# LenShustek/readtape

Hardware: AMD Instinct MI355X
Metric: Msamples/sec (all tracks) 9-trk TBIN (higher is better)
Workload: dtype i16/f32; 1 GPU; C2: synthetic 9-track 800 BPI NRZI, 781.25 kHz, 1 parmset; rows_per_gpu=101799450, rows_total=101799450, bytes_per_gpu=1832390100, parmsets=1

## Files before the change

### readtape_amd/csrc/rtfe_api.hip

```cpp
#include <hip/hip_runtime.h>

#include <limits.h>
#include <math.h>
#include <stdarg.h>
#include <stdio.h>
#include <stdlib.h>
#include <string.h>

#include <mutex>

#include "rt_frontend.h"
#include "rtfe_device.h"

#include "rtfe_sift.hip"
#include "rtfe_kernels.hip"
#include "rtfe_zeros.hip"
#include "rtfe_diffz.hip"
#include "rtfe_ww.hip"
#include "rtfe_gain.hip"
#include "rtfe_dense.hip"
#include "rtfe_pack.hip"
#include "rtfe_csv.hip"
#include "rtfe_csvout.hip"
#include "rtfe_textfile.hip"
// ... 565 lines not shown
   void t1(int k) { t1s(k, st); }
   void skip_rest() {
      unsigned mask = 0;
      for (int k = 0; k < kNumKernels; ++k) if (ran[k]) mask |= 1u << k;
      if (h->timing) h->ev_ran[evset] = mask;
      for (int k = 0; k < kNumKernels; ++k) if (!ran[k]) { t0(k); t1(k); } }
   void launch_bursts(hipStream_t s) {
      const int wpr_env = h->bursts_wpr;
      const int wpr = (wpr_env >= 1 && wpr_env <= kBrWords) ? wpr_env : kBrWords;
      const long long rounds = (L.nwords + wpr - 1) / wpr;
      if ((wpr_env > 0 || rounds >= 3) && rounds <= kBrRoundsMax && d.debug != 5) {
         hipLaunchKernelGGL(k_bursts_cnt, dim3((unsigned)rounds), dim3(1024), 0, s, (const unsigned long long *)w.qwords, L.nwords, nchunks, wpr, d.gap_chunks, a.first_is_tape_start, maxb, w.rtot);
         hipLaunchKernelGGL(k_bursts_emit, dim3((unsigned)rounds), dim3(1024), 0, s, (const unsigned long long *)w.qwords, L.nwords, nchunks, nrows, wpr, d.gap_chunks, a.first_is_tape_start, a.d_bursts, maxb, (const uint32_t *)w.rtot);
         hipLaunchKernelGGL(k_bursts_tail, dim3(1), dim3(1024), 0, s, (int)rounds, (const uint32_t *)w.rtot, nrows, (long long)a.own_rows, d.ntrks, d.gap_chunks,
                            d.cap_frac, d.nparm, (long long)a.event_capacity, a.d_bursts, maxb, w.scratch, a.d_nbursts); }
      else
         hipLaunchKernelGGL(k_bursts, dim3(1), dim3(1024), 0, s, (const unsigned long long *)w.qwords, L.nwords, nchunks, nrows, (long long)a.own_rows, d.ntrks,
                            d.gap_chunks, a.first_is_tape_start, d.cap_frac, d.nparm, (long long)a.event_capacity, a.d_bursts, maxb, w.scratch, a.d_nbursts, d.debug == 5 ? 1 : 0); }
   void launch_zones(hipStream_t s) {
      hipLaunchKernelGGL(k_zones, dim3(h->num_cus * 8), dim3(64), 0, s, h->d_dev, a.d_rows, nrows, (const rtfe_burst *)a.d_bursts, (const BurstScratch *)w.scratch, w.ctl);
      if (d.invert)
         hipLaunchKernelGGL(k_rails, dim3(h->num_cus * 8), dim3(64), 0, s, h->d_dev, a.d_rows, nrows, (const rtfe_burst *)a.d_bursts, (const BurstScratch *)w.scratch, w.ctl); }
   void launch_decode(int mode) {
      const DecodePlan dp = decode_plan(h);
      t0(kTDecode);
      hipLaunchKernelGGL(k_decode, dim3(h->num_cus * dp.per_cu), dim3(dp.threads), h->lds_bytes, st, h->d_dev, a.d_rows, nrows,
                         row_base, a.d_bursts, w.scratch, a.d_counts, a.d_events, 0xffffffffu, 0, 0, mode, w.ctl);
      t1(kTDecode); }
   void launch_sift() {
      t0(kTSift);
      const sfs_kernel_t sfs = sf_special(h);
      const int pthreads = sfs ? sfs_threads(d) : sf_threads(d), plds = sfs ? sfs_lds(d) : d.pk_lds;
      int spc = lds_wgs_per_cu(plds, 512, 32 / (pthreads / 64));
      if (h->sift_wgs >= 1 && h->sift_wgs < spc) spc = h->sift_wgs;
      if (spc < 1) spc = 1;
      long long pgrid = (long long)h->num_cus * spc;
      if (pgrid > L.ptiles) pgrid = L.ptiles;
      if (sfs) {
         for (int sc = 0; sc < d.nscreens; ++sc) {
            SfArgs sa;
            sa.rows = a.d_rows; sa.nrows = nrows; sa.ntiles = (int)L.ptiles; sa.qtile = sc == 0 ? w.qtile : nullptr; sa.dir = w.dir; sa.pool = w.pool; sa.hard = w.hard; sa.hard_cap = L.hard_cap;
            sa.hard_count = &w.scratch->hard_count; sa.dbg = w.scratch->scr; sa.hcap = d.pk_slot; sa.wave_cap = d.pk_wave_cap; sa.invert = d.invert;
            sa.quiet_i = d.quiet_i; sa.cfg = h->d_dev; sa.hi_i = d.screen[sc].sure_i;
            sa.cut = d.cut; sa.debug = d.debug; sa.defer = 1; sa.nscreens = d.nscreens; sa.sc = sc;
            const int lds_sc = sfs_lds_sc(d, sc);
            int spc_sc = lds_wgs_per_cu(lds_sc, 512, spc);
            if (h->sfs_occ[sc] >= 1 && spc_sc > h->sfs_occ[sc]) spc_sc = h->sfs_occ[sc];
            if (spc_sc < 1) spc_sc = 1;
            long long grid_sc = (long long)h->num_cus * spc_sc;
            if (grid_sc > L.ptiles) grid_sc = L.ptiles;
            hipLaunchKernelGGL(sf_special_sc(h, sc), dim3((unsigned)grid_sc), dim3(pthreads), lds_sc, st, sa); } }
      else {
         const sf_kernel_t sfk = sf_kernel(sf_wmax(d), pthreads, sf_nv(d));
         hipLaunchKernelGGL(sfk, dim3((unsigned)pgrid), dim3(pthreads), d.pk_lds, st, (const DevCfg *)h->d_dev, a.d_rows, nrows, L.ptiles,
                            w.qtile, w.dir, w.pool, w.hard, L.hard_cap, &w.scratch->hard_count, w.scratch->scr); }
      t1(kTSift); }
   void launch_streams() {
      t0(kTPrep);
      const int nlists = d.nscreens * d.ntrks;
      const int nsc = (int)((L.ptiles + 1023) / 1024);
      hipLaunchKernelGGL(k_sift_hard, dim3(h->num_cus * 16), dim3(256), 0, st, (const DevCfg *)h->d_dev, a.d_rows, nrows, (const SfHard *)w.hard, L.hard_cap,
                         (const int *)&w.scratch->hard_count, w.ovf, w.extra, w.scratch->dbg2);
      hipLaunchKernelGGL(k_pscan1, dim3(nsc), dim3(1024), 0, st, (const PeakDir *)w.dir, (const int *)w.extra, (int)L.ptiles, nlists, w.tstart, w.ctotc);
      hipLaunchKernelGGL(k_pscan2, dim3(1), dim3(1024), 0, st, nsc, nlists, (const uint32_t *)w.ctotc, w.coff, w.ctot);
      PrepArgs ppa; ppa.nlists = nlists; ppa.ntrks = d.ntrks; ppa.hcap = d.pk_slot; ppa.run = h->prep_run; ppa.mv = d.maxvolts;
      hipLaunchKernelGGL(k_prep, dim3(h->num_cus * (h->prep_wgs >= 1 && h->prep_wgs <= 4096 ? h->prep_wgs : 32)), dim3(256), 0, st, ppa, (const PeakDir *)w.dir, (const unsigned char *)w.pool, (const unsigned char *)w.ovf,
                         (const uint32_t *)w.tstart, (const uint32_t *)w.coff, (const uint32_t *)w.ctot, L.ptiles, L.ccap, w.crec, w.eref, w.work, L.work_cap, &w.scratch->prep_work);
      hipLaunchKernelGGL(k_clear, dim3(h->num_cus * 4), dim3(256), 0, st, (const unsigned long long *)w.work, L.work_cap, (const int *)&w.scratch->prep_work, (const uint32_t *)w.ctot, L.ccap, w.crec);
#ifdef RTFE_CPU_EMUL
      if (getenv("RTFE_PREP_CHECK")) hipLaunchKernelGGL(k_prep_check, dim3(1), dim3(64), 0, st, (const DevCfg *)h->d_dev, (const uint32_t *)w.ctot, L.ccap, (const CRec *)w.crec);
      if (getenv("RTFE_PREP_CHECK") && atoi(getenv("RTFE_PREP_CHECK")) > 1)
         hipLaunchKernelGGL(k_prep_shapes, dim3(1), dim3(64), 0, st, nlists, (int)d.pk_slot, h->prep_run, L.ptiles, L.ccap, (const PeakDir *)w.dir, (const unsigned char *)w.pool, (const uint32_t *)w.ctot);
#endif
      t1(kTPrep); }
   void launch_chains() {
      t0(kTGain);
      for (int mode = 0; mode < 2; ++mode) {
         if (mode == 1) t0(kTGainTail);
         hipLaunchKernelGGL(k_gain, dim3(h->num_cus * 4), dim3(64), 0, st, (const DevCfg *)h->d_dev, mode, w.cst, nrows, row_base, (const rtfe_burst *)a.d_bursts,
                            w.scratch, w.ctl, a.d_counts, a.d_events, w.chain, (const CRec *)w.crec, (const uint2 *)w.eref, (const uint32_t *)w.tstart, (const uint32_t *)w.coff, (const uint32_t *)w.ctot, L.ccap,
                            (const unsigned char *)w.pool, L.ptiles, w.segs, L.seg_cap, a.d_rows);
         if (mode == 0) {
            t1(kTGain); t0(kTGainS);
            hipLaunchKernelGGL(k_gain_seg, dim3(h->num_cus * 16), dim3(64), 0, st, (const DevCfg *)h->d_dev, (const ChainSt *)w.cst, w.scratch, (const CRec *)w.crec, L.ccap, w.segs, (const int *)&w.scratch->nsegs, L.seg_cap, w.gfire);
            hipLaunchKernelGGL(k_gain_join, dim3(h->num_cus * 2), dim3(64), 0, st, (const DevCfg *)h->d_dev, w.cst, (const rtfe_burst *)a.d_bursts, w.scratch, (const BurstCtl *)w.ctl, a.d_counts, w.chain, w.segs);
            t1(kTGainS); } }
#ifdef RTFE_CPU_EMUL
      if (getenv("RTFE_PREP_CHECK") && atoi(getenv("RTFE_PREP_CHECK")) > 1 && d.pk_seg_recs > 0)
         hipLaunchKernelGGL(k_seg_shapes, dim3(1), dim3(64), 0, st, (const DevCfg *)h->d_dev, (const ChainSt *)w.cst, (const BurstScratch *)w.scratch, (const CRec *)w.crec, L.ccap,
                            (const GsSeg *)w.segs, L.seg_cap, (const float *)w.gfire);
#endif
      t1(kTGainTail); }
   void launch_emit(hipStream_t side) {
      t0(kTEmit);
      hipStream_t se = st;
      if (side != st) { se = side; (void)hipEventRecord(h->ev_fork2, st); (void)hipStreamWaitEvent(se, h->ev_fork2, 0); }
      hipLaunchKernelGGL(k_emit, dim3(h->num_cus * 32), dim3(64), 0, se, h->d_dev, (const rtfe_burst *)a.d_bursts, (const BurstScratch *)w.scratch, (const BurstCtl *)w.ctl, (const uint32_t *)a.d_counts, a.d_events,
                         (const float *)w.chain, (const CRec *)w.crec, (const uint2 *)w.eref, L.ccap, (const unsigned char *)w.pool, (const ChainSt *)w.cst, a.d_rows, nrows, (const GsSeg *)w.segs);
      if (se != st) (void)hipEventRecord(h->ev_join2, se);
      hipLaunchKernelGGL(k_emit_seg, dim3(h->num_cus * 16), dim3(256), 0, st, (const DevCfg *)h->d_dev, (const ChainSt *)w.cst, (const BurstCtl *)w.ctl, a.d_events, (const CRec *)w.crec, (const uint2 *)w.eref, L.ccap,
                         (const unsigned char *)w.pool, (const GsSeg *)w.segs, (const int *)&w.scratch->nsegs, L.seg_cap, (const float *)w.gfire, (int)(L.max_bursts * d.nparm * d.ntrks), a.d_rows, nrows);
      if (se != st) (void)hipStreamWaitEvent(st, h->ev_join2, 0);
      hipLaunchKernelGGL(k_publish, dim3(h->num_cus < 64 ? h->num_cus : 64), dim3(256), 0, st, h->d_dev, nrows, a.d_bursts, w.scratch, w.ctl);
      if (d.nuset < d.nparm)
         hipLaunchKernelGGL(k_dup_sets, dim3(h->num_cus * 8), dim3(256), 0, st, (const DevCfg *)h->d_dev, (const rtfe_burst *)a.d_bursts, (const BurstScratch *)w.scratch, (const BurstCtl *)w.ctl, a.d_counts, a.d_events);
      t1(kTEmit); }
   void launch_peak_path() {
      const int stop_after = h->peak_stop;
      uint4 *const extra16 = ws_at<uint4>(a.d_workspace, L.extra);
      hipLaunchKernelGGL(k_scan_begin, dim3(h->num_cus * 4), dim3(256), 0, st, h->d_dev, w.scratch, extra16, (long long)((L.cst - L.extra) / 16), a.d_rows, nrows);
      launch_sift();
      hipStream_t sa = st;
      if (h->overlap && stop_after >= 99) {
         ensure_side(h);
         if (h->side) { sa = h->side; (void)hipEventRecord(h->ev_fork, st); (void)hipStreamWaitEvent(sa, h->ev_fork, 0); } }
      t0s(kTBursts, sa);
      hipLaunchKernelGGL(k_qpack, dim3(h->num_cus < 64 ? h->num_cus : 64), dim3(256), 0, sa, (const uint16_t *)w.qtile, L.ptiles, w.qwords, L.nwords);
      launch_bursts(sa);
      if (stop_after >= 3) launch_zones(sa);
      t1s(kTBursts, sa);
      if (sa != st) (void)hipEventRecord(h->ev_join, sa);
      launch_streams();
      if (sa != st) (void)hipStreamWaitEvent(st, h->ev_join, 0);
      if (stop_after < 3) return;
      launch_chains();
      if (stop_after < 4) return;
      launch_emit(sa);
      if (stop_after < 5) return;
      launch_decode(kDecodeRedo);
      if (d.adapt_floor) hipLaunchKernelGGL(k_adapt_floor, dim3(1), dim3(1), 0, st, h->d_dev, (const BurstScratch *)w.scratch); }
   void launch_dense_path() {
      (void)hipMemsetAsync(w.scratch, 0, kScratchBytes, st);
      (void)hipMemsetAsync(w.qwords, 0, (size_t)L.nwords * 8, st);
      const int dlds = (int)ds_lds_layout(d.ntrks, d.halo_rows, d.ds_pad + kDsTile + kDsRight, d.ds_up).total + 64;
      int dpc = lds_wgs_per_cu(dlds, 1024, 8);
      if (h->dseg_wgs >= 1 && h->dseg_wgs < dpc) dpc = h->dseg_wgs;
      if (dpc < 1) dpc = 1;
      long long dg = (long long)h->num_cus * dpc;
      if (dg > L.dtiles) dg = L.dtiles;
      t0(kTDseg);
      int dthreads = kDsThreads;
      if (h->dseg_threads >= 64 && h->dseg_threads <= kDsThreads) dthreads = h->dseg_threads / 64 * 64;
      unsigned char *const qbytes = ws_at<unsigned char>(a.d_workspace, L.qwords);
      hipLaunchKernelGGL(ds_kernel(h), dim3((unsigned)dg), dim3(dthreads), dlds, st, (const DevCfg *)h->d_dev, a.d_rows, nrows, L.dtiles, w.dead, qbytes, w.slot, w.scratch->scr);
      t1(kTDseg);
      t0(kTBursts);
      launch_bursts(st);
      launch_zones(st);
      t1(kTBursts);
      if (h->dense_stop < 2) return;
      t0(kTDchain);
      if (h->ds_order) hipLaunchKernelGGL(k_dorder, dim3(1), dim3(1024), 0, st, (const rtfe_burst *)a.d_bursts, (const BurstScratch *)w.scratch, w.ctl, nrows);
      int wmax = 1;
      for (int i = 0; i < d.nparm; ++i) if (d.parm[i].W > wmax) wmax = d.parm[i].W;
      const int dcache = wmax + 2 + kDcChunk < kDcCache ? ((wmax + 2 + kDcChunk + 7) & ~7) : kDcCache;
      hipLaunchKernelGGL(k_dchain, dim3(h->num_cus * (h->dchain_wgs >= 1 && h->dchain_wgs <= 64 ? h->dchain_wgs : 16)), dim3(64), (size_t)(d.ds_slot < 144 ? 144 : d.ds_slot) * 64 + (size_t)dcache * 64 * 2, st, (const DevCfg *)h->d_dev, a.d_rows, nrows, row_base, (const rtfe_burst *)a.d_bursts,
                         w.scratch, w.ctl, a.d_counts, a.d_events, (const unsigned char *)w.dead, (const unsigned char *)w.slot, L.dtiles, h->ds_order);
      hipLaunchKernelGGL(k_publish, dim3(h->num_cus < 64 ? h->num_cus : 64), dim3(256), 0, st, h->d_dev, nrows, a.d_bursts, w.scratch, w.ctl);
      t1(kTDchain);
      if (h->dense_stop < 3) return;
      launch_decode(kDecodeRedo); }
   void launch_sample_path() {
      (void)hipMemsetAsync(w.scratch, 0, kScratchBytes, st);
      const int grid = (int)(L.nwords < (long long)h->num_cus * 8 ? L.nwords : (long long)h->num_cus * 8);
      t0(kTQuiet);
      hipLaunchKernelGGL(k_quiet, dim3(grid), dim3(256), 0, st, a.d_rows, nrows, d.ntrks, d.quiet_i, w.qwords, L.nwords);
      t1(kTQuiet);
// ... 460 lines not shown
```

### readtape_amd/csrc/rtfe_gain.hip

```cpp

namespace rtfe {

__global__ void __launch_bounds__(64) k_zones(const DevCfg *__restrict__ cfgp, const int16_t *__restrict__ rows, long long nrows,
                                              const rtfe_burst *__restrict__ bursts, const BurstScratch *__restrict__ scratch, BurstCtl *__restrict__ ctl) {
   __shared__ __attribute__((aligned(16))) int16_t s_z[(kMarginRows + 2 * 50 + 2) * RTFE_MAXTRKS + 8];
   const DevCfg &cfg = *cfgp;
   const int ntrks = cfg.ntrks;
   const int nb = scratch->nbursts_total;
   for (int b = blockIdx.x; b < nb; b += gridDim.x) {
      const rtfe_burst B = bursts[b];
      long long reset;
      unsigned int bflags = B.flags;
      int status = kBurstReady;
      if (B.flags & RTFE_F_EXACT_START) { reset = B.reset_sample; status = kBurstNeedsFull; }
      else if (B.zone_end - B.zone_first < kMarginRows + 64) { reset = B.zone_end - kMarginRows; bflags |= RTFE_F_UNSAFE; status = kBurstNeedsFull; }
      else {
         const long long z0 = B.zone_end - kMarginRows;
         const long long r0 = z0 - 2 * 50 - 2 > 0 ? z0 - 2 * 50 - 2 : 0;
         const int nel = (int)(B.zone_end - r0) * ntrks;
         const long long base_e = r0 * ntrks, a0 = base_e & ~3ll, tot_e = nrows * ntrks;
         const int sh = (int)(base_e - a0), nq = (nel + sh + 3) >> 2;
         __syncthreads();
         for (int q0 = 0; q0 < nq; q0 += 64 * 16) {
            uint2 t[16];
// ... 665 lines not shown
      #pragma unroll
      for (int j = 0; j <= kGainChunk; ++j) q[j] = make_uint4(0, 0, 0, 0);
      const uint4 *rec4 = reinterpret_cast<const uint4 *>(src.rec);
      auto fetch = [&](long long i0) {
         #pragma unroll
         for (int j = 0; j <= kGainChunk; ++j) if (i0 + j < src.iend) q[j] = rec4[i0 + j]; };
      auto put = [&]() {
         #pragma unroll
         for (int j = 0; j <= kGainChunk; ++j) s_rec[j][lane] = q[j]; };
      int st2 = active ? 0 : 2;
      bool handed = false;
      if (st2 == 0) fetch(i);
      put();
      if (st2 == 0) fetch(i + kGainChunk);
      const bool prof = cfg.debug == 4 && lane == 0;
      long long pc_steps = 0, pc_gen = 0, pc_bound = 0, pn_chunks = 0, pn_gen = 0;
      for (;;) {
         long long tk0 = 0, tk1 = 0, tk2 = 0;
         if (prof) tk0 = clock64();
         int jp = 0;
         #pragma nounroll
         for (int j0 = 0; j0 < kGainChunk; j0 += 4) {
            #pragma unroll
            for (int jj = 0; jj < 4; ++jj)
               if (st2 == 0) { st2 = step(j0 + jj, i + j0 + jj); if (st2 == 0 || st2 == 3) jp = j0 + jj + 1; }
            if (__ballot(st2 == 0) == 0) break; }
         bool resync = false;
         if (prof) { tk1 = clock64(); pc_steps += tk1 - tk0; ++pn_chunks; if (__ballot(st2 == 1)) ++pn_gen; }
         if (st2 == 4) { i += jp; jp = 0; flush_notes(); rejoin(); st2 = 0; resync = true; }
         else if (st2 == 1) { i += jp; jp = 0; flush_notes(); st2 = general(); if (st2 != 2) st2 = 0; resync = true; if (st2 == 0 && mode == 0 && steady) st2 = 3; }
         else if (st2 == 0) i += kGainChunk;
         if (st2 == 3) { i += jp; flush_notes(); handed = true; st2 = 2; }
         if (prof) { tk2 = clock64(); pc_gen += tk2 - tk1; }
         if (__ballot(st2 != 2) == 0) { flush_notes(); break; }
         if (resync && st2 == 0) fetch(i);
         put();
         if (st2 == 0) fetch(i + kGainChunk);
         flush_notes();
         if (prof) pc_bound += clock64() - tk2; }
      if (prof) { atomicAdd(&scratch->dbg2[0], (unsigned long long)pc_steps); atomicAdd(&scratch->dbg2[1], (unsigned long long)pc_gen); atomicAdd(&scratch->dbg2[2], (unsigned long long)pc_bound);
                  atomicAdd(&scratch->dbg2[3], (unsigned long long)pn_chunks); atomicAdd(&scratch->dbg2[4], (unsigned long long)pn_gen); atomicAdd(&scratch->dbg2[5], 1ull); }
      if (!active) continue;
      if (handed && !failed) {
         ChainSt &cs = cst[ci];
         cs.w = w; cs.i = i; cs.c = c; cs.iend = src.iend; cs.seg0 = 0; cs.nseg = 0; cs.status = kChSteady; cs.seg_ev0 = w.nevents; cs.seg_ev1 = w.nevents; cs.pad = 0;
         cs.k.ev_index = (unsigned long long)(ev - events); cs.k.h = w.v_avg_height; cs.k.alpha = alpha; cs.k.kr = kr; cs.k.km = km; cs.k.rg_min = rg_min; cs.k.g_min = g_min;
         cs.k.W = W; cs.k.sure_i = S.sure_i; cs.k.limit32 = limit32; cs.k.amp_on = amp_on ? 1 : 0; cs.k.sl = sl; cs.k.pad = 0;
         {  const long long len = src.iend > i ? src.iend - i : 0;
            const int SR = cfg.pk_seg_recs;
            int nseg = len <= 0 ? 0 : (int)((len + SR - 1) / SR);
            int seg0 = nseg > 0 ? atomicAdd(&scratch->nsegs, nseg) : 0;
            if ((long long)seg0 + nseg > seg_cap) nseg = 0;
            cs.seg0 = seg0; cs.nseg = nseg;
            for (int sg = 0; sg < nseg; ++sg) {
               GsSeg &o = segs[seg0 + sg];
               o.chain = ci; o.sidx = sg; o.first = i + (long long)sg * SR; o.end = sg + 1 == nseg ? src.iend : i + (long long)(sg + 1) * SR; o.stands = 0;
               o.ev_index = (unsigned long long)(ev - events); o.reset = reset; o.h = w.v_avg_height; o.sl = sl; } }
         for (int k = 0; k < 10; ++k) cs.heights[k] = heights[k];
         if (w.v_avg_height > 0) atomicMax(&scratch->min_height_key, 0x7fffffff - (int)__float_as_uint(w.v_avg_height));
         if (n_slow) atomicAdd(&scratch->dbg[1], (unsigned long long)n_slow);
         if (w.nevents > n_slow) atomicAdd(&scratch->dbg[0], (unsigned long long)(w.nevents - n_slow));
         continue; }
      cst[ci].status = kChDone;
      if (mode == 0) { cst[ci].seg_ev0 = 0; cst[ci].seg_ev1 = 0; cst[ci].pad = 0; }
      if (rejoined) cst[ci].pad = 1;
      n_fast = w.nevents - n_slow - (mode == 1 ? cst[ci].w.nevents : 0u);
      if (n_fast) atomicAdd(&scratch->dbg[0], (unsigned long long)n_fast);
      if (n_slow) atomicAdd(&scratch->dbg[1], (unsigned long long)n_slow);
      if (failed) { atomicExch(&ctl[b].status, (int)kBurstNeedsFull); atomicAdd(&scratch->why[why & 7], 1ull); }
      counts[((size_t)b * cfg.nparm + pidx) * ntrks + trk] = w.nevents < cap ? w.nevents : cap;
      chain_h[(size_t)b * nwalk + wi] = w.v_avg_height;
      if (mode == 0 && !agc_off && w.peakcount > 15 && w.v_avg_height_count == 0 && w.v_avg_height > 0) atomicMax(&scratch->min_height_key, 0x7fffffff - (int)__float_as_uint(w.v_avg_height));
      if (w.flags & ~(unsigned)RTFE_F_SCREEN_UNDERFLOW) atomicOr(&ctl[b].bflags, w.flags & ~(unsigned)RTFE_F_SCREEN_UNDERFLOW); } }

constexpr int kGsRegs = 8, kGsDepth = 1;
constexpr int kGsPitch = kGsRegs + 1;
__global__ void __launch_bounds__(64) k_gain_seg(const DevCfg *__restrict__ cfgp, const ChainSt *__restrict__ cst, BurstScratch *__restrict__ scratch,
                                                 const CRec *__restrict__ crec, long long ccap, GsSeg *__restrict__ segs, const int *__restrict__ nsegs_p, long long seg_cap, float *__restrict__ gfire) {
   __shared__ uint4 s_rec[64 * kGsPitch];
   const int lane = threadIdx.x;
   const int nsegs = (int)min((long long)*nsegs_p, seg_cap);
   const int nchains = scratch->nbursts * cfgp->nparm * cfgp->ntrks;
   const int S = cfgp->pk_seg_recs;
   const bool prof = cfgp->debug == 6 && threadIdx.x == 0;
   long long pt0 = 0, pt_setup = 0, pt_steps = 0, pn_chunks = 0, pn_items = 0;
   for (int sbase = blockIdx.x * 64; sbase < nsegs; sbase += gridDim.x * 64) {
      const int si = sbase + lane < nsegs ? sbase + lane : nsegs - 1;
      if (prof) { pt0 = clock64(); ++pn_items; }
      GsSeg sg = segs[si];
      bool active = sbase + lane < nsegs && (unsigned)sg.chain < (unsigned)nchains;
      if (!active) sg.chain = 0;
      const ChainSt &cs = cst[sg.chain];
      active = active && cs.status == kChSteady && si >= cs.seg0 && si < cs.seg0 + cs.nseg && sg.sidx == si - cs.seg0;
      if (!active) { sg.sidx = 0; sg.first = 0; sg.end = 0; }
      const GsConst K = cs.k;
      const int W = K.W, sure_i = K.sure_i, limit32 = K.limit32;
      const bool amp_on = K.amp_on != 0;
      const float h = K.h, alpha = K.alpha, beta = 1 - K.alpha, kr = K.kr, km = K.km, rg_min = K.rg_min, g_min = K.g_min;
      const uint4 *rec4 = reinterpret_cast<const uint4 *>(crec + (size_t)K.sl * ccap);
      float *gout = gfire + (size_t)si * S;
      float g = cs.w.agc_gain, vlt = cs.w.v_lasttop, vlb = cs.w.v_lastbot;
      int rise_hi = cs.w.rise_hi, min_lo = cs.w.min_lo, min_hi = cs.w.min_hi;
      int c = sg.sidx == 0 ? (int)cs.c : 0;
      long long i = sg.first;
      if (sg.sidx > 0) { i = sg.first - cfgp->parm[(sg.chain % (cfgp->nparm * cfgp->ntrks)) / cfgp->ntrks].seg_warm; if (i < cs.i) i = cs.i; }
      unsigned int nev = 0;
      if (prof) pt_setup += clock64() - pt0;
      auto walk = [&](const long long to, const bool own, const bool act) -> long long {
         bool run = act && i < to;
         const int piece = lane & 7, sub = lane >> 3;
         float hq = h / (vlt - vlb);
         bool lhpos = vlt - vlb > 0;
         uint4 q[kGsDepth][kGsRegs];
         auto fetch = [&](uint4 (&dst)[kGsRegs], const long long at) {
            const unsigned long long mine = reinterpret_cast<unsigned long long>(rec4 + at);
            const int left = run ? (int)((to - at) < kGsRegs ? (to - at > 0 ? to - at : 0) : kGsRegs) : 0;
            #pragma unroll
            for (int k = 0; k < kGsRegs; ++k) {
               const int src = 8 * k + sub;
               const unsigned lo = (unsigned)__shfl((int)(unsigned)mine, src), hi = (unsigned)__shfl((int)(unsigned)(mine >> 32), src);
               const int n = __shfl(left, src);
               dst[k] = make_uint4(0, kCrBad, 0, 0);
               if (piece < n) dst[k] = reinterpret_cast<const uint4 *>(((unsigned long long)hi << 32) | lo)[piece]; } };
         #pragma unroll
         for (int dd = 0; dd < kGsDepth; ++dd) fetch(q[dd], i + dd * kGsRegs);
         bool more = __ballot(run) != 0ull;
         while (more) {
            #pragma unroll
            for (int dd = 0; dd < kGsDepth; ++dd) {
               if (!more) break;
               long long tc0 = 0;
               if (prof) { tc0 = clock64(); ++pn_chunks; }
               #pragma unroll
               for (int k = 0; k < kGsRegs; ++k) s_rec[(8 * k + sub) * kGsPitch + piece] = q[dd][k];
               rtfe_wave_sync();
               fetch(q[dd], i + kGsDepth * kGsRegs);
               int adv = 0;
               const bool ran = run;
               float gb[kGsRegs];
               #pragma unroll
               for (int j = 0; j < kGsRegs; ++j) {
                  const uint4 r = s_rec[lane * kGsPitch + j];
                  const bool inr = run && i + j < to;
                  const int pos = (int)r.x;
                  const uint32_t w0 = r.y;
                  const bool bad = w0 & kCrBad;
                  const bool dead = bad ? pos + kSfTile + W < c : pos + W - 2 < c;
                  const int val = (int)(int16_t)(r.z & 0xffffu);
                  const bool top = !(w0 & 0x800u);
                  const int a = top ? val : -val;
                  const bool ampdead = (!bad && r.z != 0xffff8000u && amp_on && a <= min_lo) || crec_weak_dead(w0, rise_hi - 5);
                  const int f = pos + (int)((w0 >> 12) & 63u), fl = f + (int)((w0 >> 18) & 15u);
                  const bool fire = (w0 & kCrClear) && c <= f && fl < limit32 && rise_hi <= crec_level(w0, sure_i) && (!amp_on || a >= min_hi) && g >= g_min;
                  const float v = __uint_as_float(r.w);
                  const float lh_f = top ? v - vlb : vlt - v;
                  const float q_f = h / lh_f;
                  float g2 = alpha * hq + beta * g;
                  g2 = g2 > 2.0f ? 2.0f : g2;
                  g2 = lhpos ? g2 : g;
                  const float rg = fast_rcp(g2);
                  const bool ok = inr && !dead && !ampdead && fire && g2 > 0 && rg >= rg_min;
                  gb[j] = ok ? g : 0.0f;
                  nev += ok ? 1u : 0u;
                  c = ok ? pos + W + 1 : c;
                  vlt = ok && top ? v : vlt; vlb = ok && !top ? v : vlb;
                  hq = ok ? q_f : hq; lhpos = ok ? lh_f > 0 : lhpos;
                  g = ok ? g2 : g;
                  const int rr = (int)(kr * rg), mm = (int)(km * rg);
                  rise_hi = ok ? rr + 3 : rise_hi; min_lo = ok ? mm - 2 : min_lo; min_hi = ok ? mm + 3 : min_hi;
                  const bool on = inr && (dead || ampdead || ok || !own);
                  if (run && !on) { run = false; adv = j; } }
               if (run) adv = kGsRegs;
               if (own && ran) {
                  float4 *o4 = reinterpret_cast<float4 *>(gout + (i - sg.first));
                  o4[0] = make_float4(gb[0], gb[1], gb[2], gb[3]); o4[1] = make_float4(gb[4], gb[5], gb[6], gb[7]); }
               rtfe_wave_sync();
               i += adv;
               if (i >= to) run = false;
               more = __ballot(run) != 0ull;
               if (prof) pt_steps += clock64() - tc0; } }
         return i; };
      walk(sg.first, false, active && sg.sidx > 0);
      i = sg.first; nev = 0;
      GsState s0; s0.g = g; s0.vlt = vlt; s0.vlb = vlb; s0.c = c; s0.rise_hi = rise_hi; s0.min_lo = min_lo; s0.min_hi = min_hi;
      const long long at = walk(sg.end, true, active);
      if (active) {
         GsSeg &o = segs[si];
         o.at_first = s0;
         o.at_end.g = g; o.at_end.vlt = vlt; o.at_end.vlb = vlb; o.at_end.c = c; o.at_end.rise_hi = rise_hi; o.at_end.min_lo = min_lo; o.at_end.min_hi = min_hi;
         o.stop = at > sg.end ? sg.end : at; o.cnt = (int)nev; } }
   if (prof) { atomicAdd(&scratch->dbg2[0], (unsigned long long)pt_setup); atomicAdd(&scratch->dbg2[1], (unsigned long long)pt_steps);
               atomicAdd(&scratch->dbg2[3], (unsigned long long)pn_chunks); atomicAdd(&scratch->dbg2[4], (unsigned long long)pn_items); } }

__global__ void __launch_bounds__(64) k_gain_join(const DevCfg *__restrict__ cfgp, ChainSt *__restrict__ cst, const rtfe_burst *__restrict__ bursts, BurstScratch *__restrict__ scratch,
                                                  const BurstCtl *__restrict__ ctl, uint32_t *__restrict__ counts, float *__restrict__ chain_h, GsSeg *__restrict__ segs) {
   const DevCfg &cfg = *cfgp;
   const int ntrks = cfg.ntrks, nwalk = cfg.nparm * ntrks;
   const int nchains = chain_count(cfg, scratch->nbursts);
   for (int cu = blockIdx.x * 64 + threadIdx.x; cu < nchains; cu += gridDim.x * 64) {
      const ChainIx cx_ = chain_ix(cfg, cu);
      const int ci = cx_.ci, b = cx_.b, wi = cx_.wi, pidx = cx_.pidx, trk = cx_.trk;
      if (ctl[b].status != kBurstReady || cst[ci].status != kChSteady) continue;
      ChainSt &cs = cst[ci];
      const unsigned int cap = bursts[b].event_cap;
      const unsigned int nev0 = cs.w.nevents;
      unsigned int nev = nev0;
      long long resume = cs.i;
      GsState st; st.g = cs.w.agc_gain; st.vlt = cs.w.v_lasttop; st.vlb = cs.w.v_lastbot; st.c = (int)cs.c; st.rise_hi = cs.w.rise_hi; st.min_lo = cs.w.min_lo; st.min_hi = cs.w.min_hi;
      bool through = cs.nseg > 0;
      for (int k = 0; k < cs.nseg; ++k) {
         GsSeg &sg = segs[cs.seg0 + k];
         if (!gs_same(sg.at_first, st) || (unsigned long long)nev + (unsigned)sg.cnt > cap) { through = false; break; }
         sg.stands = 1; sg.evoff = nev;
         nev += (unsigned)sg.cnt; st = sg.at_end; resume = sg.stop;
         if (sg.stop < sg.end) { through = false; break; } }
      if (nev > nev0) atomicAdd(&scratch->dbg[0], (unsigned long long)(nev - nev0));
      cs.w.agc_gain = st.g; cs.w.v_lasttop = st.vlt; cs.w.v_lastbot = st.vlb; cs.w.v_top = st.vlt; cs.w.v_bot = st.vlb;
      cs.w.peakcount += (int)(nev - nev0); cs.w.nevents = nev; cs.i = resume; cs.c = st.c;
      cs.seg_ev0 = nev0; cs.seg_ev1 = nev;
      if (through) {
         cs.status = kChDone;
         counts[((size_t)b * cfg.nparm + pidx) * ntrks + trk] = nev < cap ? nev : cap;
         chain_h[(size_t)b * nwalk + wi] = cs.w.v_avg_height; }
      else cs.status = kChGeneral; } }
#ifdef RTFE_CPU_EMUL
__global__ void __launch_bounds__(64) k_seg_shapes(const DevCfg *__restrict__ cfgp, const ChainSt *__restrict__ cst, const BurstScratch *__restrict__ scratch, const CRec *__restrict__ crec, long long ccap,
                                                   const GsSeg *__restrict__ segs, long long seg_cap, const float *__restrict__ gfire) {
   if (blockIdx.x != 0 || threadIdx.x != 0) return;
   const DevCfg &cfg = *cfgp;
   const int nsegs = (int)min((long long)scratch->nsegs, seg_cap), S = cfg.pk_seg_recs, nwalk = cfg.nparm * cfg.ntrks;
   const int nchains = scratch->nbursts * nwalk;
   long long planned = 0, standing = 0, refused = 0, stopped = 0, rejoined = 0, nc_first = 0, nc_last = 0, nc_warm = 0, nc_near = 0, round_edge = 0, weak = 0, unknown = 0;
   auto notclear = [](const CRec &r) { return !(r.w0 & kCrClear) || (r.w0 & kCrWeak) || r.w1 == 0xffff8000u; };
   for (int si = 0; si < nsegs; ++si) {
      const GsSeg &sg = segs[si];
      if ((unsigned)sg.chain >= (unsigned)nchains) continue;
      const ChainSt &cs = cst[sg.chain];
      if (si < cs.seg0 || si >= cs.seg0 + cs.nseg || sg.sidx != si - cs.seg0 || sg.end <= sg.first) continue;
      ++planned;
      const CRec *r = crec + (size_t)sg.sl * ccap;
      const long long i0 = segs[cs.seg0].first;
      if (sg.sidx == 0) rejoined += cs.status == kChDone && cs.pad == 1;
      else {
         const GsSeg &pv = segs[si - 1];
         refused += pv.stands == 1 && pv.stop == pv.end && sg.stands != 1 && !gs_same(sg.at_first, pv.at_end);
         const int warm = cfg.parm[(sg.chain % nwalk) / cfg.ntrks].seg_warm;
         for (long long i = sg.first - warm < i0 ? i0 : sg.first - warm; i < sg.first; ++i) nc_warm += notclear(r[i]);
         for (long long i = sg.first - 4 < i0 ? i0 : sg.first - 4; i < sg.first + 5 && i < sg.end; ++i) nc_near += notclear(r[i]);
         nc_first += notclear(r[sg.first]); }
      if (si + 1 < cs.seg0 + cs.nseg) nc_last += notclear(r[sg.end - 1]);
      for (long long i = sg.first; i < sg.end; ++i) { weak += (r[i].w0 & kCrWeak) != 0; unknown += r[i].w1 == 0xffff8000u; }
      if (sg.stands != 1) continue;
      ++standing;
      stopped += sg.stop < sg.end;
      const long long n_own = sg.stop - sg.first;
      for (long long k = 63; k + 1 < n_own && k + 1 < S; k += 64) round_edge += (gfire[(size_t)si * S + k] != 0.0f) + (gfire[(size_t)si * S + k + 1] != 0.0f); }
   const long long back = __atomic_exchange_n(&g_seg_back_cross, 0ll, __ATOMIC_RELAXED), back_any = __atomic_exchange_n(&g_seg_back_any, 0ll, __ATOMIC_RELAXED);
   fprintf(stderr, "seg_shapes: recs %d planned %lld standing %lld refused %lld stopped %lld rejoined %lld nc_first %lld nc_last %lld nc_warm %lld nc_near %lld back_any %lld back_cross %lld round_edge %lld weak %lld unknown %lld\n",
           S, planned, standing, refused, stopped, rejoined, nc_first, nc_last, nc_warm, nc_near, back_any, back, round_edge, weak, unknown); }
#endif
__device__ __forceinline__ rtfe_event emit_event(const DevCfg &cfg, const DevParm &P, Walker &wk, const CRec &r, const uint16_t *eend, const MarSrc &ms, float gain, int W, int d, long long reset,
                                                 int trk, int pidx, float mv) {
   const Run u = run_decode(r.w0, r.w1, (long long)r.pos);
   wk.agc_gain = gain; wk.flags = 0;
   update_thresholds(wk, P, cfg.lsb_per_volt);
   long long n = u.f + u.nlead;
   for (int j = u.nlead - 1; j >= 0; --j) if (rise_pass(wk, u.top, u.val, run_margin(ms, u, eend, j), mv)) n = u.f + j;
   const int ld = (int)(u.pos - n) + W;
   const int iprev = u.top ? u.val - u.dprev : u.val + u.dprev, inext = u.top ? u.val - u.dnext : u.val + u.dnext;
   const int adjcode = refine_code(&cfg, u.val, iprev, inext, gain, u.top);
   const float val = r.volt;
   rtfe_event e;
   e.sample = (uint32_t)(n + d - reset);
   e.v_peak = (cfg.invert && val == 0.0f) ? -0.0f : val;
// ... 147 lines not shown
```

Before: 81600 Msamples/s.

## Restructure gain segment walk loop and size its grid from segment capacity

The k_gain_seg inner loop now tracks a remaining-count instead of comparing 64-bit positions. It also loads all shared-memory records into registers before issuing the next prefetch, replaces short-circuit logic with branch-free bitwise predicates, and inlines the weak-level checks. Output pointers advance incrementally, and the at_first state is written straight to global memory. The launch grid is now sized from seg_cap, capped at 32 workgroups per CU instead of a fixed 16, which adds parallelism but raises register pressure from the extra record array.

```diff
diff --git a/readtape_amd/csrc/rtfe_api.hip b/readtape_amd/csrc/rtfe_api.hip
--- a/readtape_amd/csrc/rtfe_api.hip
+++ b/readtape_amd/csrc/rtfe_api.hip
@@ -671,7 +671,8 @@
                             (const unsigned char *)w.pool, L.ptiles, w.segs, L.seg_cap, a.d_rows);
          if (mode == 0) {
             t1(kTGain); t0(kTGainS);
-            hipLaunchKernelGGL(k_gain_seg, dim3(h->num_cus * 16), dim3(64), 0, st, (const DevCfg *)h->d_dev, (const ChainSt *)w.cst, w.scratch, (const CRec *)w.crec, L.ccap, w.segs, (const int *)&w.scratch->nsegs, L.seg_cap, w.gfire);
+            const long long gs_wgs = (L.seg_cap + 63) / 64, gs_max = (long long)h->num_cus * 32;
+            hipLaunchKernelGGL(k_gain_seg, dim3((unsigned)(gs_wgs < 1 ? 1 : (gs_wgs > gs_max ? gs_max : gs_wgs))), dim3(64), 0, st, (const DevCfg *)h->d_dev, (const ChainSt *)w.cst, w.scratch, (const CRec *)w.crec, L.ccap, w.segs, (const int *)&w.scratch->nsegs, L.seg_cap, w.gfire);
             hipLaunchKernelGGL(k_gain_join, dim3(h->num_cus * 2), dim3(64), 0, st, (const DevCfg *)h->d_dev, w.cst, (const rtfe_burst *)a.d_bursts, w.scratch, (const BurstCtl *)w.ctl, a.d_counts, w.chain, w.segs);
             t1(kTGainS); } }
 #ifdef RTFE_CPU_EMUL
diff --git a/readtape_amd/csrc/rtfe_gain.hip b/readtape_amd/csrc/rtfe_gain.hip
--- a/readtape_amd/csrc/rtfe_gain.hip
+++ b/readtape_amd/csrc/rtfe_gain.hip
@@ -771,7 +771,7 @@
    const int nsegs = (int)min((long long)*nsegs_p, seg_cap);
    const int nchains = scratch->nbursts * cfgp->nparm * cfgp->ntrks;
    const int S = cfgp->pk_seg_recs;
-   const bool prof = cfgp->debug == 6 && threadIdx.x == 0;
+   const bool prof = cfgp->debug == 6;
    long long pt0 = 0, pt_setup = 0, pt_steps = 0, pn_chunks = 0, pn_items = 0;
    for (int sbase = blockIdx.x * 64; sbase < nsegs; sbase += gridDim.x * 64) {
       const int si = sbase + lane < nsegs ? sbase + lane : nsegs - 1;
@@ -787,7 +787,7 @@
       const bool amp_on = K.amp_on != 0;
       const float h = K.h, alpha = K.alpha, beta = 1 - K.alpha, kr = K.kr, km = K.km, rg_min = K.rg_min, g_min = K.g_min;
       const uint4 *rec4 = reinterpret_cast<const uint4 *>(crec + (size_t)K.sl * ccap);
-      float *gout = gfire + (size_t)si * S;
+      float4 *gout = reinterpret_cast<float4 *>(gfire + (size_t)si * S);
       float g = cs.w.agc_gain, vlt = cs.w.v_lasttop, vlb = cs.w.v_lastbot;
       int rise_hi = cs.w.rise_hi, min_lo = cs.w.min_lo, min_hi = cs.w.min_hi;
       int c = sg.sidx == 0 ? (int)cs.c : 0;
@@ -797,22 +797,23 @@
       if (prof) pt_setup += clock64() - pt0;
       auto walk = [&](const long long to, const bool own, const bool act) -> long long {
          bool run = act && i < to;
+         int left = run ? (int)(to - i < 0x40000000ll ? to - i : 0x40000000ll) : 0;
          const int piece = lane & 7, sub = lane >> 3;
          float hq = h / (vlt - vlb);
          bool lhpos = vlt - vlb > 0;
          uint4 q[kGsDepth][kGsRegs];
-         auto fetch = [&](uint4 (&dst)[kGsRegs], const long long at) {
+         auto fetch = [&](uint4 (&dst)[kGsRegs], const long long at, const int left_at) {
             const unsigned long long mine = reinterpret_cast<unsigned long long>(rec4 + at);
-            const int left = run ? (int)((to - at) < kGsRegs ? (to - at > 0 ? to - at : 0) : kGsRegs) : 0;
+            const int n_at = run ? (left_at < kGsRegs ? (left_at > 0 ? left_at : 0) : kGsRegs) : 0;
             #pragma unroll
             for (int k = 0; k < kGsRegs; ++k) {
                const int src = 8 * k + sub;
                const unsigned lo = (unsigned)__shfl((int)(unsigned)mine, src), hi = (unsigned)__shfl((int)(unsigned)(mine >> 32), src);
-               const int n = __shfl(left, src);
+               const int n = __shfl(n_at, src);
                dst[k] = make_uint4(0, kCrBad, 0, 0);
                if (piece < n) dst[k] = reinterpret_cast<const uint4 *>(((unsigned long long)hi << 32) | lo)[piece]; } };
          #pragma unroll
-         for (int dd = 0; dd < kGsDepth; ++dd) fetch(q[dd], i + dd * kGsRegs);
+         for (int dd = 0; dd < kGsDepth; ++dd) fetch(q[dd], i + dd * kGsRegs, left - dd * kGsRegs);
          bool more = __ballot(run) != 0ull;
          while (more) {
             #pragma unroll
@@ -823,24 +824,31 @@
                #pragma unroll
                for (int k = 0; k < kGsRegs; ++k) s_rec[(8 * k + sub) * kGsPitch + piece] = q[dd][k];
                rtfe_wave_sync();
-               fetch(q[dd], i + kGsDepth * kGsRegs);
                int adv = 0;
                const bool ran = run;
                float gb[kGsRegs];
+               uint4 rq[kGsRegs];
+               #pragma unroll
+               for (int j = 0; j < kGsRegs; ++j) rq[j] = s_rec[lane * kGsPitch + j];
+               fetch(q[dd], i + kGsDepth * kGsRegs, left - kGsDepth * kGsRegs);
                #pragma unroll
                for (int j = 0; j < kGsRegs; ++j) {
-                  const uint4 r = s_rec[lane * kGsPitch + j];
-                  const bool inr = run && i + j < to;
+                  const uint4 r = rq[j];
+                  const bool inr = run & (j < left);
                   const int pos = (int)r.x;
                   const uint32_t w0 = r.y;
-                  const bool bad = w0 & kCrBad;
-                  const bool dead = bad ? pos + kSfTile + W < c : pos + W - 2 < c;
+                  const bool bad = (w0 & kCrBad) != 0;
+                  const bool dead = pos + (bad ? kSfTile + W : W - 2) < c;
                   const int val = (int)(int16_t)(r.z & 0xffffu);
                   const bool top = !(w0 & 0x800u);
                   const int a = top ? val : -val;
-                  const bool ampdead = (!bad && r.z != 0xffff8000u && amp_on && a <= min_lo) || crec_weak_dead(w0, rise_hi - 5);
+                  const int lvl = (int)((w0 >> 3) & 255u);
+                  const bool weak = (w0 & kCrWeak) != 0;
+                  const bool weakdead = weak & (lvl != 255) & (16 * lvl <= rise_hi - 5);
+                  const bool ampdead = (!bad & (r.z != 0xffff8000u) & amp_on & (a <= min_lo)) | weakdead;
                   const int f = pos + (int)((w0 >> 12) & 63u), fl = f + (int)((w0 >> 18) & 15u);
-                  const bool fire = (w0 & kCrClear) && c <= f && fl < limit32 && rise_hi <= crec_level(w0, sure_i) && (!amp_on || a >= min_hi) && g >= g_min;
+                  const int level = weak ? 16 * lvl - 16 : sure_i;
+                  const bool fire = ((w0 & kCrClear) != 0) & (c <= f) & (fl < limit32) & (rise_hi <= level) & (!amp_on | (a >= min_hi)) & (g >= g_min);
                   const float v = __uint_as_float(r.w);
                   const float lh_f = top ? v - vlb : vlt - v;
                   const float q_f = h / lh_f;
@@ -848,37 +856,34 @@
                   g2 = g2 > 2.0f ? 2.0f : g2;
                   g2 = lhpos ? g2 : g;
                   const float rg = fast_rcp(g2);
-                  const bool ok = inr && !dead && !ampdead && fire && g2 > 0 && rg >= rg_min;
+                  const bool ok = inr & !dead & !ampdead & fire & (g2 > 0) & (rg >= rg_min);
                   gb[j] = ok ? g : 0.0f;
                   nev += ok ? 1u : 0u;
                   c = ok ? pos + W + 1 : c;
-                  vlt = ok && top ? v : vlt; vlb = ok && !top ? v : vlb;
+                  vlt = (ok & top) ? v : vlt; vlb = (ok & !top) ? v : vlb;
                   hq = ok ? q_f : hq; lhpos = ok ? lh_f > 0 : lhpos;
                   g = ok ? g2 : g;
                   const int rr = (int)(kr * rg), mm = (int)(km * rg);
                   rise_hi = ok ? rr + 3 : rise_hi; min_lo = ok ? mm - 2 : min_lo; min_hi = ok ? mm + 3 : min_hi;
-                  const bool on = inr && (dead || ampdead || ok || !own);
-                  if (run && !on) { run = false; adv = j; } }
-               if (run) adv = kGsRegs;
+                  run = inr & (dead | ampdead | ok | !own);
+                  adv += run ? 1 : 0; }
                if (own && ran) {
-                  float4 *o4 = reinterpret_cast<float4 *>(gout + (i - sg.first));
-                  o4[0] = make_float4(gb[0], gb[1], gb[2], gb[3]); o4[1] = make_float4(gb[4], gb[5], gb[6], gb[7]); }
+                  gout[0] = make_float4(gb[0], gb[1], gb[2], gb[3]); gout[1] = make_float4(gb[4], gb[5], gb[6], gb[7]); gout += 2; }
                rtfe_wave_sync();
-               i += adv;
-               if (i >= to) run = false;
+               i += adv; left -= adv;
+               run = run & (left > 0);
                more = __ballot(run) != 0ull;
                if (prof) pt_steps += clock64() - tc0; } }
          return i; };
       walk(sg.first, false, active && sg.sidx > 0);
       i = sg.first; nev = 0;
-      GsState s0; s0.g = g; s0.vlt = vlt; s0.vlb = vlb; s0.c = c; s0.rise_hi = rise_hi; s0.min_lo = min_lo; s0.min_hi = min_hi;
+      if (active) { GsState &s0 = segs[si].at_first; s0.g = g; s0.vlt = vlt; s0.vlb = vlb; s0.c = c; s0.rise_hi = rise_hi; s0.min_lo = min_lo; s0.min_hi = min_hi; }
       const long long at = walk(sg.end, true, active);
       if (active) {
          GsSeg &o = segs[si];
-         o.at_first = s0;
          o.at_end.g = g; o.at_end.vlt = vlt; o.at_end.vlb = vlb; o.at_end.c = c; o.at_end.rise_hi = rise_hi; o.at_end.min_lo = min_lo; o.at_end.min_hi = min_hi;
-         o.stop = at > sg.end ? sg.end : at; o.cnt = (int)nev; } }
-   if (prof) { atomicAdd(&scratch->dbg2[0], (unsigned long long)pt_setup); atomicAdd(&scratch->dbg2[1], (unsigned long long)pt_steps);
+         o.stop = at; o.cnt = (int)nev; } }
+   if (prof && threadIdx.x == 0) { atomicAdd(&scratch->dbg2[0], (unsigned long long)pt_setup); atomicAdd(&scratch->dbg2[1], (unsigned long long)pt_steps);
                atomicAdd(&scratch->dbg2[3], (unsigned long long)pn_chunks); atomicAdd(&scratch->dbg2[4], (unsigned long long)pn_items); } }
 
 __global__ void __launch_bounds__(64) k_gain_join(const DevCfg *__restrict__ cfgp, ChainSt *__restrict__ cst, const rtfe_burst *__restrict__ bursts, BurstScratch *__restrict__ scratch,
```

Result: faster. 82490 Msamples/s (median of 6 runs) (+1.1%).
